# sieste/greb-climate-model

Hardware: AMD Instinct MI355X
Metric: simulated-years/sec at 96x48 grid (ensemble aggregate); diffusion HBM GB/s vs roofline (higher is better)
Workload: dtype f32; 1 GPU; 96x48 GREB ensemble, 512 members/GPU x 1 GPU, CO2 sweep 280-1120 ppm, 32 scenario years after 1 flux-correction year, dt=12h, dt_crcl=0.5h; members_per_gpu=512, arithmetic=fast, gather=none (1 GPU)

## Files before the change

greb_climate_model_amd/abi.py:

```python
from __future__ import annotations

import ctypes as C
import math

import numpy as np

NSTEP_YR = 730
NVAR_OUT = 5
F_STRICT = 1
F_MULTILAUNCH = 2
F_ROW_STRIPS = 4
F_NO_PERSISTENT = 8
F_PERSISTENT = 16
RUN_DEVICE_OUT = 1
D_REGIONS, D_ZONAL, D_ANNUAL = 1, 2, 4
D_MAX_REGIONS = 15
C_MEAN, C_SEASONS, C_TREND, C_RESPONSE = 1, 2, 4, 8
S_MEAN, S_VAR, S_RANGE, S_QUANTILES = 1, 2, 4, 8
ENS_MAX_GROUPS, ENS_MAX_PROBS, ENS_MAX_SORTED = 64, 16, 4096
L_COEF, L_RSS = 1, 2
LIN_MAX_TERMS = 64
GRAM_MAX_BLOCKS, GRAM_MAX_USED = 16, 1024
X_NAMES = ("GREB_X_NO_ICE", "GREB_X_NO_HYDRO", "GREB_X_NO_DEEP_OCEAN", "GREB_X_LW_LINEAR_VAPOR", "GREB_X_NO_CIRCULATION",
           "GREB_X_NO_VAPOR_TRANSPORT", "GREB_X_VAPOR_DIFFUSION_ONLY", "GREB_X_SST_PLUS1")
BUDGET_NAMES = ("sw", "LW_surf", "LWair_down", "LW_abs", "Q_sens", "Q_lat", "Q_lat_air", "dq_eva", "dq_rain", "dT_ocean",
                "dTo", "dTa_crcl", "dq_crcl")
NBUDGET = len(BUDGET_NAMES)
(B_SW, B_LW_SURF, B_LWAIR_DOWN, B_LW_ABS, B_Q_SENS, B_Q_LAT, B_Q_LAT_AIR, B_DQ_EVA, B_DQ_RAIN, B_DT_OCEAN, B_DTO,
 B_DTA_CRCL, B_DQ_CRCL) = range(NBUDGET)
# ... 223 lines not shown
```

greb_climate_model_amd/csrc/greb_batched.cpp:

```cpp
#include "greb_host.h"

#include <cstring>
#include <mutex>

using namespace greb;
using namespace greb::host;

#define HIP_TRY0(expr) HIP_TRY(nullptr, expr)

namespace {
int batched_common(const greb_params* p, int nx, int ny, int batch, int device) {
  if (!p || !grid_ok(nx, ny) || batch < 1) return fail(nullptr, GREB_E_INVALID, "batched: bad argument");
  return use_device("batched: ", device);
}

struct TabCache {
  struct Entry { int device; RowTables* dev; RowTables host; unsigned long long used; };
  std::mutex mu;
  std::vector<Entry> entries;
  unsigned long long clock = 0;
  static constexpr size_t kMax = 32;
} g_tab_cache;
}

// ... 87 lines not shown
  a.flux_phase = flux_phase != 0;
  a.xsw = switches ? 1u : 0u;
  if (budget) a.bsum = a.brec = budget_words;
  if (on_sets) { a.bsets = sets; a.bset_m = set_of_member; }
  if (forced || (on_sets && !flux_phase)) a.force_m = force_words;
  if (select_variant(a, variant) != hipSuccess) return fail(nullptr, GREB_E_INVALID, "step_variant: no launch carries this combination");
  return 0;
}

int greb_step_variants(unsigned* out, int capacity) {
  if (capacity < 0 || (capacity > 0 && !out)) return fail(nullptr, GREB_E_INVALID, "step_variants: bad argument");
  for (int i = 0; i < kNVariants && i < capacity; ++i) out[i] = kVariants[i];
  return kNVariants;
}

int greb_member_deal_cover(int strict, int* counts) {
  if (!counts) return fail(nullptr, GREB_E_INVALID, "member_deal_cover: bad argument");
  member_deal_cover(strict != 0, counts);
  return 0;
}

int greb_member_lds_table(int strict, int* records, int capacity) {
  if (capacity < 0 || (capacity > 0 && !records)) return fail(nullptr, GREB_E_INVALID, "member_lds_table: bad argument");
  return member_lds_table(strict != 0, records, capacity);
}

int greb_member_lds_map(int* words8) {
  if (!words8) return fail(nullptr, GREB_E_INVALID, "member_lds_map: bad argument");
  member_lds_map(words8);
  return 0;
// ... 102 lines not shown
```

greb_climate_model_amd/csrc/greb_engine.cpp:

```cpp
#include "greb_host.h"

#include <cmath>
#include <cstdio>
#include <cstring>
#include <mutex>
#include <new>

using namespace greb;
using namespace greb::host;
using StripPlan = greb_engine::StripPlan;

thread_local std::string greb::host::g_last_error;

static int nint_f(float x) { return (int)lroundf(x); }

void greb::host::compute_row_tables(const greb_params& p, float kappa, int nx, int ny, RowTables& g) {
  std::memset(&g, 0, sizeof(g));
  const float dlon = 360.f / (float)nx, dlat = 180.f / (float)ny;
  const float deg = 2.f * p.pi * 6.371e6f / 360.f;
  const float dx = dlon, dy = dlat, dyy = dy * deg;
  const float dtc = (float)p.dt_crcl;
  g.dif_ccy = kappa * dtc / (dyy * dyy);
  g.adv_ccy = dtc / dyy / 2.f;
  for (int k = 0; k < ny; ++k) {
// ... 58 lines not shown
  MemberArgs a{};
  a.nx = e->nx; a.ny = e->ny; a.np = e->np;
  a.z_topo = e->z_topo; a.glacier = e->glacier; a.sw_solar = e->sw_solar;
  a.tclim = e->tclim; a.qclim = e->qclim; a.uclim = e->uclim; a.vclim = e->vclim;
  a.mldclim = e->mldclim; a.cldclim = e->cldclim; a.swetclim = e->swetclim;
  a.toclim = e->toclim; a.z_ocean = e->z_ocean; a.wz_air = e->wz_air; a.wz_vapor = e->wz_vapor;
  a.state = e->state; a.acc = e->acc; a.corr = e->corr; a.corr_index = e->corr_index;
  a.tabs = e->tabs; a.tab_index = e->tab_index; a.phys = e->phys;
  a.nsub = nsub_of(e->p);
  a.nsub = tuning_int("GREB_DEBUG_NSUB", a.nsub);
  a.co2_flux = e->p.co2_flux;
  a.ipx = e->p.ipx; a.ipy = e->p.ipy;
  a.xsw = e->xsw_uniform ? e->xsw : 0u;
  a.xsw_m = e->xsw_uniform ? nullptr : e->xsw_dev;
  a.co2_flux_m = e->co2_flux_dev;
  a.stamps = e->stamps;
  a.dbg = tuning_int("GREB_DEBUG_PHYS", 0);
  unsigned all = GREB_X_NO_CIRCULATION;
  for (unsigned x : e->h_xsw) all &= x;
  if (all) a.nsub = 0;
  if (e->members_on_sets > 0) { a.bsets = e->bsets_dev; a.bset_m = e->bset_dev; }
  else if (e->bound[0].frec) a.bsets = e->bsets_dev;
  return a;
}

static void apply_forcing(const greb_engine* e, MemberArgs& a) {
  if (e->forced_members <= 0 && e->members_on_sets > 0) a.force_m = e->neutral_force_dev;
  if (e->forced_members <= 0) return;
  a.force_m = e->force_dev;
  a.f_space = e->f_space; a.f_season = e->f_season; a.f_solar = e->f_solar;
}
// ... 76 lines not shown
  std::lock_guard<std::mutex> lock(g_slots.mu);
  long long members = 0, taken = 0;
  SlotLedger::Entry* mine = nullptr;
  for (auto& x : g_slots.entries) {
    if (x.device != e->device) continue;
    members += x.members;
    if (x.e == e) mine = &x; else taken += x.granted;
  }
  if (!mine) return 0;
  const long long share = (long long)device_slots * mine->members / std::max<long long>(1, members);
  mine->granted = (int)std::max<long long>(0, std::min<long long>(share, device_slots - taken));
  return mine->granted;
}

static int check_circulation(greb_engine* e) {
  for (auto& kv : e->plans) {
    unsigned d[5] = {0, 0, 0, 0, 0};
    const int rc = circ_rows_status(kv.second.circ, d);
    if (rc == -1) {
      char buf[384];
      std::snprintf(buf, sizeof(buf),
                    "circulation launch given up: task %u waited more than %.1f s in sub-step %u for a neighbouring strip "
                    "(its count read %u, wanted %u) -- the launch was not resident as a whole (another process on the "
                    "device?); results are invalid, recreate the engine with GREB_F_NO_PERSISTENT",
                    d[0], kCircSpinTicks / 1e8, d[1], d[2], d[3]);
      return fail(e, GREB_E_STATE, buf);
    }
    if (rc) return fail(e, GREB_E_STATE, "circulation launch: status word unreadable");
  }
  return 0;
// ... 5 lines not shown
    static const int slots_per_cu = tuning_int("GREB_CIRC_SLOTS_PER_CU", kStepRowsSlotsPerCu);
    if (e->slots_granted < 0) e->slots_granted = ledger_grant(e, e->cus * std::min(slots_per_cu, kStepRowsSlotsPerCu));
    HIP_TRY(e, circ_rows_make_order(e->h_tabs.data(), e->h_tab_index.data(), nrun, e->ny, e->slots_granted, &p.circ));
  }
  p.form = p.circ.n == 0 ? 1 : (e->call == greb_engine::kCallAlways ? 2 : 0);
  if (p.form != 2) {
    static const int step_slots = tuning_int("GREB_STEP_SLOTS_PER_CU", kStepRowsSlotsPerCu);
    HIP_TRY(e, step_rows_make_tasks(e->h_tabs.data(), e->h_tab_index.data(), nrun, e->ny, e->cus * step_slots, &p.step_tasks,
                                    &p.n_step, p.head));
  }
  if (p.form == 0)
    for (hipEvent_t& ev : p.ev) HIP_TRY(e, hipEventCreate(&ev));
  return 0;
}

int greb::host::run_year(greb_engine* e, const MemberArgs& a, int nrun) {
  if (e->fused) {
    HIP_TRY(e, launch_member_kernel(a, nrun, e->strict, e->stream));
    return 0;
  }
  const size_t np = (size_t)e->np;
  StripPlan* plan = nullptr;
  if (e->strips && a.nsub > 0) {
    auto it = e->plans.find(nrun);
    if (it == e->plans.end()) {
      StripPlan p;
      if (int rc = make_strip_plan(e, nrun, p)) { free_plan(p); return rc; }
      it = e->plans.emplace(nrun, p).first;
    }
    plan = &it->second;
  }
  static const int steps = tuning_int("GREB_DEBUG_NSTEPS", kNT);
  bool trial = plan && plan->form == 0 && steps >= 16;
// ... 303 lines not shown
    c.p.da_ice = pick(p->da_ice, overrides[m].da_ice);
    c.p.a_no_ice = pick(p->a_no_ice, overrides[m].a_no_ice);
    c.p.a_cloud = pick(p->a_cloud, overrides[m].a_cloud);
    c.p.kappa = pick(p->kappa, overrides[m].kappa);
  }
  return create_engine("greb_engine_create", p, nx, ny, f, n_members, members.data(), device, flags, out);
}

int greb_engine_destroy(greb_engine* e) {
  if (!e) return 0;
  (void)hipSetDevice(e->device);
  void* ptrs[] = {e->z_topo, e->glacier, e->sw_solar, e->tclim, e->qclim, e->uclim, e->vclim, e->mldclim,
                  e->cldclim, e->swetclim, e->toclim, e->z_ocean, e->wz_air, e->wz_vapor, e->state, e->acc,
                  e->corr, e->corr_index, e->tab_index, e->tabs, e->phys, e->co2_dev, e->monthly_dev, e->yearly_dev,
                  e->Xa, e->Xb, e->red, e->W2, e->xsw_dev, e->co2_flux_dev, e->diag_out, e->diag_reg, e->clim_out, e->ens_out, e->lin_out, e->gram_out, e->derive_out, e->bsum, e->budget_dev,
                  e->f_space, e->f_season, e->f_solar, e->force_dev, e->bsets_dev, e->bset_dev, e->neutral_force_dev};
  for (void* q : ptrs) if (q) (void)hipFree(q);
  for (const auto& b : e->bound) if (b.frec) (void)hipFree(b.frec);
  for (size_t k = 1; k < e->bound.size(); ++k)
    for (int i = 0; i < kBoundaryFields; ++i) if (e->bound[k].own[i]) (void)hipFree(e->bound[k].dev[i]);
  for (auto& kv : e->plans) free_plan(kv.second);
  if (e->call != greb_engine::kCallNever) ledger_release(e);
  for (int i = 0; i < 2; ++i) {
    if (e->ev_done[i]) (void)hipEventDestroy(e->ev_done[i]);
    if (e->ev_free[i]) (void)hipEventDestroy(e->ev_free[i]);
  }
  if (e->copy_stream) (void)hipStreamDestroy(e->copy_stream);
  if (e->stream) (void)hipStreamDestroy(e->stream);
  delete e;
  return 0;
}
// ... 56 lines not shown
    int n = 0;
    for (const auto& b : e->bound) n += b.frec != nullptr;
    std::snprintf(buf, sizeof(buf), ", \"forcing_records\": {\"sets\": %d, \"bytes\": %zu}", n, (size_t)n * kFrBytes);
    s += buf;
  }
  {
    unsigned v;
    auto family = [&v](const MemberArgs& a) { return select_variant(a, &v) == hipSuccess ? variant_family(v) : "none"; };
    MemberArgs flux = base_args(e), scenario = base_args(e);
    flux.flux_phase = 1;
    apply_forcing(e, scenario);
    std::snprintf(buf, sizeof(buf), ", \"kernel_family\": {\"flux_correction\": \"%s\", \"scenario\": \"%s\"}", family(flux),
                  family(scenario));
    s += buf;
  }
  if (e->call != greb_engine::kCallNever) {
    std::snprintf(buf, sizeof(buf), ", \"wavefront_slots_granted\": %d, \"circulation\": [", e->slots_granted);
    s += buf;
    bool first = true;
    for (const auto& kv : e->plans) {
      const StripPlan& p = kv.second;
      std::snprintf(buf, sizeof(buf), "%s{\"members_run\": %d, \"tasks_of_one_launch_per_call\": %d, \"form\": \"%s\", \"trial_ms_per_3_steps\": [%.4f, %.4f]}",
                    first ? "" : ", ", kv.first, p.circ.n,
                    p.circ.n == 0 ? "one launch per sub-step (slots)" : (p.form == 2 ? "one launch per call" : (p.form == 1 ? "one launch per sub-step" : "undecided")),
                    p.ms_substep, p.ms_call);
      s += buf;
      first = false;
    }
    s += "]";
  }
// ... 18 lines not shown
}

int greb_engine_set_corrections(greb_engine* e, int member, const float* corr, const float* state5) {
  if (!e || member < -1 || member >= e->nm) return fail(e, GREB_E_INVALID, "set_corrections: bad argument");
  HIP_TRY(e, hipSetDevice(e->device));
  const size_t n = (size_t)3 * kNT * e->np, s5 = (size_t)5 * e->np;
  const int m0 = member < 0 ? 0 : member, m1 = member < 0 ? e->nm : member + 1;
  for (int m = m0; m < m1; ++m) {
    const size_t ci = e->shared_corr ? 0 : (size_t)m;
    if (corr && (ci == (size_t)m || m == m0)) HIP_TRY(e, hipMemcpy(e->corr + ci * n, corr, n * sizeof(float), hipMemcpyHostToDevice));
    if (state5) HIP_TRY(e, hipMemcpy(e->state + (size_t)m * s5, state5, s5 * sizeof(float), hipMemcpyHostToDevice));
  }
  return 0;
}

int greb_engine_set_state(greb_engine* e, int member, const float* state5) {
  if (!state5) return fail(e, GREB_E_INVALID, "set_state: bad argument");
  return greb_engine_set_corrections(e, member, nullptr, state5);
}

}
```

greb_climate_model_amd/csrc/greb_host.h:

```cpp
#pragma once
#include "../../include/greb_engine.h"

#include <hip/hip_runtime.h>

#include <functional>
#include <map>
#include <string>
#include <vector>

#include "greb_kernels.h"

struct greb_engine {
  greb_params p{};
  int nx = 0, ny = 0, np = 0, nm = 0, device = 0;
  bool strict = false;
  unsigned xsw = 0;
  std::vector<unsigned> h_xsw;
  bool xsw_uniform = true;
  unsigned* xsw_dev = nullptr;
  float* co2_flux_dev = nullptr;
  int n_phys_sets = 1;
  bool shared_corr = true;
  bool fused = true;
  float *Xa = nullptr, *Xb = nullptr, *red = nullptr, *W2 = nullptr;
// ... 47 lines not shown
  int cus = 0;
  int slots_granted = -1;
  struct StripPlan {
    greb::RowsTask* step_tasks = nullptr;
    int n_step = 0;
    greb::RowsTask head[greb::kStepHeadTasks] = {};
    greb::CircOrder circ;
    int form = 0;
    float ms_substep = 0.f, ms_call = 0.f;
    hipEvent_t ev[3] = {nullptr, nullptr, nullptr};
  };
  std::map<int, StripPlan> plans;
  std::vector<greb::Phys> h_phys;
  long long it_flux = 0;
  long long it_scnr = 0;
  unsigned long long* stamps = nullptr;
  std::string last_error;
};

namespace greb {
namespace host {

extern thread_local std::string g_last_error;
int fail(greb_engine* e, int code, const std::string& msg);

#define HIP_STEP(e, who, what, expr)                                                          \
  do {                                                                                        \
    hipError_t _err = (expr);                                                                 \
    if (_err != hipSuccess)                                                                   \
      return fail((e), (int)_err, std::string(who) + (what) + ": " + hipGetErrorString(_err)); \
// ... 86 lines not shown
```

greb_climate_model_amd/csrc/greb_kernels.h:

```cpp
#pragma once
#include <hip/hip_runtime.h>

#include <cstdlib>
#include <utility>
#include <vector>

#include "greb_device.h"

namespace greb {

constexpr int kNT = 730;

#ifdef GREB_TUNING
inline int tuning_int(const char* name, int dflt) {
  const char* e = getenv(name);
  return e ? atoi(e) : dflt;
}
#else
constexpr int tuning_int(const char*, int dflt) { return dflt; }
#endif

constexpr int kMaxDynamicLds = 160 * 1024;

struct MemberForcing {
// ... 13 lines not shown
constexpr int kMaxBoundarySets = 16;

constexpr int kFrNx = 96, kFrNy = 48;
enum { kFrZtopo, kFrGlacier, kFrZocean, kFrWzAir, kFrStaticFields,
       kFrTclim = kFrStaticFields, kFrCld, kFrMld, kFrMldPrev, kFrSwet, kFrWind, kFrFields };
constexpr int kFrStepFields = kFrFields - kFrStaticFields;
constexpr unsigned forcing_record_offset(int row, int field, int lon) {
  return field < kFrStaticFields ? ((unsigned)row * kFrStaticFields + (unsigned)field) * kFrNx + (unsigned)lon
                                 : ((unsigned)row * kFrStepFields + (unsigned)(field - kFrStaticFields)) * kFrNx + (unsigned)lon;
}
constexpr unsigned kFrStaticFloats = forcing_record_offset(kFrNy, 0, 0), kFrStepFloats = forcing_record_offset(kFrNy, kFrStaticFields, 0);
constexpr size_t kFrBytes = ((size_t)kFrStaticFloats + (size_t)kNT * kFrStepFloats) * sizeof(float);
static_assert(forcing_record_offset(0, kFrFields - 1, 0) * sizeof(float) <= 4095 && forcing_record_offset(0, kFrStaticFields - 1, 0) * sizeof(float) <= 4095,
              "a field's offset must fit the immediate of a global load");
static_assert(kFrBytes < (1ull << 31), "offsets into a record are 32-bit");

struct MemberArgs {
  int nx, ny, np;
  const float *z_topo, *glacier, *sw_solar;
  const float *tclim, *qclim, *uclim, *vclim, *mldclim, *cldclim, *swetclim;
  const float *toclim, *z_ocean, *wz_air, *wz_vapor;
  float* state;
  float* acc;
  float* corr;
  const int* corr_index;
  const RowTables* tabs;
  const int* tab_index;
  const Phys* phys;
  int flux_phase;
  long long it0;
// ... 12 lines not shown
  unsigned xsw;
  unsigned long long* stamps;
  int dbg;
  const unsigned* xsw_m;
  const float* co2_flux_m;
  float* bsum;
  float* brec;
  int brec_years;
  int brec_year0;
  const MemberForcing* force_m;
  const float* f_space;
  const float* f_season;
  const float* f_solar;
  const BoundarySet* bsets;
  const int* bset_m;
};

constexpr int kSetTableEntries = kMaxBoundarySets + 1;
constexpr size_t kSetTableBytes = kSetTableEntries * (sizeof(BoundarySet) + sizeof(const float*));
inline const float** set_table_records(BoundarySet* table) { return (const float**)(table + kSetTableEntries); }

enum { kBsw, kBLWsurf, kBLWdown, kBLWabs, kBQsens, kBQlat, kBQlatAir, kBdqEva, kBdqRain, kBdTocean, kBdTo, kBdTaCrcl, kBdqCrcl, kNBudget };

enum : unsigned { kVFlux = 1, kVExp = 2, kVBudget = 4, kVForce = 8, kVBound = 16 };
constexpr bool variant_valid(unsigned v) {
  const bool flux = v & kVFlux, exp = v & kVExp, budget = v & kVBudget, force = v & kVForce, bound = v & kVBound;
  return v < 32u && !(budget && flux) && (!force || (exp && !flux)) && (!bound || (exp && (flux || force)));
}
constexpr unsigned kVariants[] = {0u, kVFlux, kVExp, kVFlux | kVExp, kVBudget, kVExp | kVBudget, kVExp | kVForce,
                                  kVExp | kVBudget | kVForce, kVFlux | kVExp | kVBound, kVExp | kVForce | kVBound,
// ... 18 lines not shown
  return (v & kVBound) ? "boundary" : (v & kVForce) ? "forcing" : (v & kVExp) ? "switches" : "default";
}
template <template <bool, unsigned> class Family, size_t... I>
auto pick_variant(bool strict, unsigned v, std::index_sequence<I...>) {
  decltype(Family<false, 0u>::kernel()) k = nullptr;
  ((kVariants[I] == v ? (void)(k = strict ? Family<true, kVariants[I]>::kernel() : Family<false, kVariants[I]>::kernel()) : (void)0), ...);
  return k;
}
template <template <bool, unsigned> class Family>
auto pick_variant(bool strict, unsigned v) { return pick_variant<Family>(strict, v, std::make_index_sequence<kNVariants>{}); }

bool member_layout_supported(const RowTables& tab, int nx, int ny);
void member_deal_cover(bool strict, int* counts);
int member_lds_table(bool strict, int* out, int capacity);
void member_lds_map(int* words8);
hipError_t launch_member_kernel(const MemberArgs& a, int n_members, bool strict, hipStream_t s);
hipError_t launch_pack_forcing(const BoundarySet& b, float* rec, hipStream_t s);
hipError_t launch_circulation_g96(const float* X, const float* wz, const float* u, const float* v, float* dX,
                                  const RowTables* tab_dev, int batch, int nsub, bool strict, hipStream_t s);

hipError_t launch_diffusion(const float* T1, const float* wz, float* dX, const RowTables* tab_dev,
                            const RowTables& tab_host, int nx, int ny, int batch, bool strict, hipStream_t s);
bool rows_supported(const RowTables& t, int nx, int ny);
struct RowsTask { int field, rows; };
constexpr int kRowsUp = 1 << 20;
struct RowsTuning {
  int chain_target;
  int chain_span;
  int parts[4];
  int level_tasks[4];
};
// ... 72 lines not shown
```

greb_climate_model_amd/csrc/greb_member.hip:

```cpp
#include <cstdlib>

#include "greb_kernels.h"
#include "greb_pair.h"
#include "greb_physics_step.h"
#include "greb_stencil.h"

namespace greb {

constexpr int NX = 96, NY = 48, NQ = 24, NP = 4608;
constexpr int kThreads = 512;
constexpr int RS = 2 * NX + 16;
constexpr int XB = (NY + 2) * RS;
constexpr int kOffX = RS;
constexpr int kOffW = 2 * XB + RS;
constexpr int kOffWX = 3 * XB;
constexpr int kOffWY = kOffWX + NP;
constexpr int kOffRowK = kOffWY + NP;
constexpr int kRowKCsDif = 7;
constexpr int kLdsFloats = kOffRowK + NY * kRowKWords;
constexpr size_t kLdsBytes = (size_t)kLdsFloats * sizeof(float);

bool member_layout_supported(const RowTables& t, int nx, int ny) {
  if (nx != NX || ny != NY) return false;
  for (int k = 0; k < NY; ++k) {
// ... 612 lines not shown
            const float y = vq[j].v[e];
            vq[j].v[e] = (k == 1 ? y > 0.f : y < 0.f) ? 3.f * y : y;
          }
        }
      }
      st4(lds + kOffWX + 4 * i, uq[j]); st4(lds + kOffWY + 4 * i, vq[j]);
    }
  }
  (void)tab;
}

template <bool STRICT>
struct Circ {
  __device__ __forceinline__ void init(lfloat* lds, const float* wz_air, const float* wz_vapor,
                                       const RowTables* __restrict__ tab) {
    for (int i = threadIdx.x; i < 6 * RS; i += kThreads) {
      const int g = i / RS, o = i % RS;
      lds[(g >> 1) * XB + (g & 1) * (NY + 1) * RS + o] = 0.f;
    }
    stage_row_consts(lds + kOffRowK, *tab, 0, NY);
    if (!STRICT)
      for (int k = threadIdx.x; k < NY; k += blockDim.x)
        lds[kOffRowK + k * kRowKWords + kRowKCsDif] = lds[kOffRowK + k * kRowKWords] * 0.05f;
    for (int i = threadIdx.x; i < NP / 4; i += kThreads)
      st8(lds + kOffW + (i / NQ) * RS, i % NQ, zip(ld4(wz_air + 4 * i), ld4(wz_vapor + 4 * i)));
  }

  template <int WAVE, bool NOT_CALM>
  __device__ __forceinline__ void role_loop(lfloat* lds, int cur, int nsub, int lane, int dbg, bool calm_runtime
#ifdef GREB_TUNING
                                            , bool stamp, unsigned long long& busy
#endif
  ) {
    const bool calm_q = NOT_CALM ? false : calm_runtime;
    constexpr bool kPolar = is_polar_wave<STRICT>(WAVE);
    BulkTasks tasks;
    BulkSigns signs;
    QuadChain quad;
    if constexpr (!kPolar) tasks = make_tasks<STRICT, WAVE>(lane);
// ... 68 lines not shown
    st4(dX + fo + 4 * i, f4{{a.v[0] - b.v[0], a.v[1] - b.v[1], a.v[2] - b.v[2], a.v[3] - b.v[3]}});
  }
}

hipError_t launch_circulation_g96(const float* X, const float* wz, const float* u, const float* v, float* dX,
                                  const RowTables* tab_dev, int batch, int nsub, bool strict, hipStream_t s) {
  auto kern = strict ? circulation_g96_kernel<true> : circulation_g96_kernel<false>;
  hipError_t e = hipFuncSetAttribute(reinterpret_cast<const void*>(kern),
                                     hipFuncAttributeMaxDynamicSharedMemorySize, (int)kLdsBytes);
  if (e != hipSuccess) return e;
  hipLaunchKernelGGL(kern, dim3(batch), dim3(kThreads), kLdsBytes, s, X, wz, u, v, dX, tab_dev, nsub,
                     tuning_int("GREB_DEBUG_SKIP", 0));
  return hipGetLastError();
}

template <bool STRICT, unsigned V>
__global__ __launch_bounds__(kThreads) void member_kernel(MemberArgs a) {
  constexpr bool FLUX = V & kVFlux, EXP = V & kVExp, BUDGET = V & kVBudget, FORCE = V & kVForce, BOUND = V & kVBound;
  extern __shared__ __align__(16) float lds_raw[];
  lfloat* lds = (lfloat*)lds_raw;
  const int m = blockIdx.x, tid = threadIdx.x;
  float* state = a.state + (size_t)m * 5 * NP;
  float* acc = a.acc + (size_t)m * 6 * NP;
  float* corr = a.corr + (size_t)a.corr_index[m] * 3 * kNT * NP;
  const RowTables* tab = a.tabs + a.tab_index[m];

#ifdef GREB_TUNING
  for (int i = 0; i < (a.dbg >> 8) * (m & 7); ++i) __builtin_amdgcn_s_sleep(16);
#endif
  Circ<STRICT> circ;
  const int bset = member_bset<BOUND>(a, m);
  {
    const BoundPtr B = member_boundary<BOUND>(a, bset);
    circ.init(lds, BOUND ? (const float*)B->wz_air : a.wz_air, BOUND ? (const float*)B->wz_vapor : a.wz_vapor, tab);
  }
  for (int i = tid; i < NP / 4; i += kThreads)
    st8(lds + kOffX + (i / NQ) * RS, i % NQ, zip(ld4(state + NP + 4 * i), ld4(state + 3 * NP + 4 * i)));
  int cur = 0;
  const unsigned xsw = EXP ? member_switches(a, m) : 0u;
  const int nsub = (EXP && (xsw & kXNoCirc)) ? 0 : a.nsub;
  const bool q_dif_only = EXP && (xsw & kXQDiffOnly) && !(xsw & kXNoQTransport);
  const float co2_flux = FLUX ? (a.co2_flux_m ? a.co2_flux_m[m] : a.co2_flux) : 0.f;
  __syncthreads();
#ifdef GREB_TUNING
  const bool stamp = a.stamps != nullptr;
  unsigned long long st_wind = 0, st_circ = 0, st_busy = 0, st_phys = 0;
  const unsigned long long st_c0 = stamp ? __builtin_amdgcn_s_memtime() : 0, st_r0 = stamp ? __builtin_amdgcn_s_memrealtime() : 0;
#define GREB_STAMP(var) const unsigned long long var = stamp ? __builtin_amdgcn_s_memtime() : 0
#else
#define GREB_STAMP(var)
#endif

#pragma unroll 1
  for (int s = 0; s < a.nsteps; ++s) {
    const long long it = a.it0 + s;
    const StepClock ck = step_clock<FLUX>(a, it, NP);
    const int ityr = ck.ityr, yr_rel = ck.yr_rel;
    const size_t off = ck.off;

    GREB_STAMP(t_a);
    {
      const BoundPtr B = member_boundary<BOUND>(a, bset);
      stage_winds<STRICT, EXP && !STRICT>(lds, (BOUND ? (const float*)B->uclim : a.uclim) + off,
                                          (BOUND ? (const float*)B->vclim : a.vclim) + off, tab);
    }
    __syncthreads();
    GREB_STAMP(t_b);

#ifdef GREB_TUNING
// ... 63 lines not shown
        }
      }
    }
    __syncthreads();
#ifdef GREB_TUNING
    if (stamp) {
      const unsigned long long t_d = __builtin_amdgcn_s_memtime();
      st_wind += t_b - t_a; st_circ += t_c - t_b; st_phys += t_d - t_c;
    }
#endif
  }
#ifdef GREB_TUNING
  if (stamp && (tid & 63) == 0) {
    unsigned long long* o = a.stamps + ((size_t)m * (kThreads / 64) + (tid >> 6)) * 8;
    o[0] = __builtin_amdgcn_s_memtime() - st_c0; o[1] = __builtin_amdgcn_s_memrealtime() - st_r0;
    o[2] = st_wind; o[3] = st_circ; o[4] = st_busy; o[5] = st_phys; o[6] = (unsigned long long)a.nsteps; o[7] = (unsigned long long)nsub;
  }
#endif
}

static_assert(kFrNx == NX && kFrNy == NY, "the forcing record is the fused kernel's grid");
__global__ __launch_bounds__(256) void pack_forcing_kernel(BoundarySet b, float* __restrict__ rec) {
  const unsigned i = blockIdx.x * 256u + threadIdx.x;
  if (i >= (unsigned)kNT * NP) return;
  const unsigned step = i / NP, p = i - step * NP, row = p / NX, lon = p - row * NX;
  const unsigned prev = step > 0 ? step - 1 : kNT - 1;
  const float zt = b.z_topo[p];
  if (step == 0) {
    float* o = rec + forcing_record_offset((int)row, 0, (int)lon);
    o[forcing_record_offset(0, kFrZtopo, 0)] = zt;
    o[forcing_record_offset(0, kFrGlacier, 0)] = b.glacier[p];
    o[forcing_record_offset(0, kFrZocean, 0)] = b.z_ocean[p];
    o[forcing_record_offset(0, kFrWzAir, 0)] = b.wz_air[p];
// ... 3 lines not shown
  o[forcing_record_offset(0, kFrCld, 0)] = b.cldclim[i];
  o[forcing_record_offset(0, kFrMld, 0)] = b.mldclim[i];
  o[forcing_record_offset(0, kFrMldPrev, 0)] = b.mldclim[(size_t)prev * NP + p];
  o[forcing_record_offset(0, kFrSwet, 0)] = b.swetclim[i];
  o[forcing_record_offset(0, kFrWind, 0)] = wind_speed<false>(b.uclim[i], b.vclim[i], zt);
}

hipError_t launch_pack_forcing(const BoundarySet& b, float* rec, hipStream_t s) {
  hipLaunchKernelGGL(pack_forcing_kernel, dim3((kNT * NP + 255) / 256), dim3(256), 0, s, b, rec);
  return hipGetLastError();
}

template <bool STRICT, unsigned V>
struct MemberFamily { static auto kernel() { return &member_kernel<STRICT, V>; } };

hipError_t launch_member_kernel(const MemberArgs& a, int n_members, bool strict, hipStream_t s) {
  if (a.nx != NX || a.ny != NY) return hipErrorInvalidValue;
  if (!strict && !a.bsets) return hipErrorInvalidValue;
  unsigned v;
  if (hipError_t e = select_variant(a, &v); e != hipSuccess) return e;
  const auto kern = pick_variant<MemberFamily>(strict, v);
  if (!kern) return hipErrorInvalidValue;
  hipError_t e = hipFuncSetAttribute(reinterpret_cast<const void*>(kern),
                                     hipFuncAttributeMaxDynamicSharedMemorySize, (int)kLdsBytes);
  if (e != hipSuccess) return e;
  hipLaunchKernelGGL(kern, dim3(n_members), dim3(kThreads), kLdsBytes, s, a);
  return hipGetLastError();
}

}
```

greb_climate_model_amd/csrc/greb_stencil.h:

```cpp
#pragma once
#include "greb_chain6.h"
#include "greb_device.h"

namespace greb {

__device__ __forceinline__ void wave_lds_sync() {
  asm volatile("s_waitcnt lgkmcnt(0)" ::: "memory");
  __builtin_amdgcn_wave_barrier();
}

struct Rows {
  const lfloat* base;
  int r0, nx;
  __device__ __forceinline__ const lfloat* row(int k) const { return base + (k - r0) * nx; }
};

struct QuadIn {
  float T[12], w[12];
  f4 T0, w0, Tm2, Tm1, Tp1, Tp2, wm2, wm1, wp1, wp2;
};


struct RowK {
  float dif_cc;
  float adv_cc;
  float dif_ccy, adv_ccy;
  int sub;
  int dif_time2, adv_time2;
};
constexpr int kRowKWords = 8;
__device__ __forceinline__ void stage_row_consts(lfloat* dst, const RowTables& tab, int k_begin, int k_end) {
  for (int k = k_begin + threadIdx.x; k < k_end; k += blockDim.x) {
    const int sub = tab.subcycled[k];
    lfloat* d = dst + (k - k_begin) * kRowKWords;
    d[0] = sub ? tab.dif_ccx2[k] : tab.dif_ccx[k];
    d[1] = sub ? tab.adv_ccx2[k] : tab.adv_ccx[k];
    d[2] = tab.dif_ccy; d[3] = tab.adv_ccy;
    d[4] = __int_as_float(sub); d[5] = __int_as_float(tab.dif_time2[k]); d[6] = __int_as_float(tab.adv_time2[k]);
    d[7] = 0.f;
  }
}
__device__ __forceinline__ RowK row_consts(const lfloat* src, int k) {
  const f4 a = ld4(src + k * kRowKWords), b = ld4(src + k * kRowKWords + 4);
  RowK r;
  r.dif_cc = a.v[0]; r.adv_cc = a.v[1]; r.dif_ccy = a.v[2]; r.adv_ccy = a.v[3];
  r.sub = __float_as_int(b.v[0]); r.dif_time2 = __float_as_int(b.v[1]); r.adv_time2 = __float_as_int(b.v[2]);
  return r;
// ... 325 lines not shown
```

greb_climate_model_amd/engine.py:

```python
from __future__ import annotations

import ctypes as C
import json
import os

import numpy as np

from . import abi, build, workload

_lib = None


class GrebError(RuntimeError):
    def __init__(self, code: int, msg: str):
        super().__init__(f"greb engine error {code}: {msg}")
        self.code = code


_lib_path = build.LIB


def use_tuning_build() -> None:
    global _lib_path
    if _lib is not None:
# ... 36 lines not shown
           "greb_clim_create", "greb_clim_destroy", "greb_clim_add_year_dev", "greb_clim_finish_dev", "greb_engine_run_clim",
           "greb_ens_create", "greb_ens_destroy", "greb_ens_reduce_dev", "greb_engine_run_ens",
           "greb_lin_create", "greb_lin_destroy", "greb_lin_reduce_dev", "greb_engine_run_lin",
           "greb_forcing_record_offset", "greb_forcing_record_field_bytes", "greb_forcing_record_step_floats",
           "greb_forcing_record_bytes", "greb_forcing_record_field_name", "greb_engine_get_forcing_record",
           "greb_forcing_record_field_static", "greb_forcing_record_static_floats",
           "greb_diag_create_vars", "greb_clim_create_vars", "greb_budget_combine_dev", "greb_engine_run_budget_diag",
           "greb_engine_run_budget_clim", "greb_engine_run_budget_ens", "greb_engine_run_budget_lin",
           "greb_gram_create", "greb_gram_destroy", "greb_gram_reduce_dev", "greb_engine_run_gram", "greb_engine_run_budget_gram",
           "greb_cross_create", "greb_cross_destroy", "greb_cross_add_year_dev", "greb_cross_finish_dev", "greb_engine_run_cross",
           "greb_engine_run_budget_cross",
           "greb_reg_create", "greb_reg_destroy", "greb_reg_add_year_dev", "greb_reg_finish_dev", "greb_engine_run_reg",
           "greb_engine_run_budget_reg",
           "greb_derive_create", "greb_derive_destroy", "greb_derive_uses_budget", "greb_derive_apply_dev",
           "greb_engine_run_derived_diag", "greb_engine_run_derived_clim", "greb_engine_run_derived_ens", "greb_engine_run_derived_lin",
           "greb_engine_run_derived_gram", "greb_engine_run_derived_cross", "greb_engine_run_derived_reg"]


def _check(rc: int, h=None):
    if rc != 0:
        msg = lib().greb_engine_last_error(h)
        raise GrebError(rc, msg.decode() if msg else "")


def device_info(device: int = 0) -> dict:
    return json.loads(lib().greb_device_info(device).decode())


def budget_name(i: int) -> str | None:
    f = lib().greb_budget_name
    f.restype = C.c_char_p
# ... 85 lines not shown
                 (abi.F_ROW_STRIPS if row_strips else 0) |
                 (0 if persistent is None else (abi.F_PERSISTENT if persistent else abi.F_NO_PERSISTENT)))
        if members is not None:
            rc = L.greb_engine_create_members(C.byref(self.params), inp.nx, inp.ny, C.byref(fields), n_members,
                                              member_configs(self.params, members), device, flags, C.byref(self.h))
        else:
            rc = L.greb_engine_create(C.byref(self.params), inp.nx, inp.ny, C.byref(fields), n_members, ov, device, flags,
                                      C.byref(self.h))
        if rc != 0:
            msg = L.greb_engine_last_error(self.h).decode()
            if self.h:
                L.greb_engine_destroy(self.h)
                self.h = None
            raise GrebError(rc, msg)

    def describe(self) -> dict:
        f = lib().greb_engine_describe
        f.restype = C.c_char_p
        return json.loads(f(self.h).decode())

    def close(self):
        if getattr(self, "h", None):
            lib().greb_engine_destroy(self.h)
            self.h = None

    def __del__(self):
        try:
            self.close()
        except Exception:
            pass
# ... 262 lines not shown
def substep_launch_order(params, nx, ny, n_members, kappa=None):
    params = params if params is not None else params_default()
    kap = None if kappa is None else np.ascontiguousarray(kappa, np.float32)
    kp = None if kap is None else kap.ctypes.data_as(C.POINTER(C.c_float))
    f = lib().greb_substep_launch_order
    n = f(C.byref(params), nx, ny, n_members, kp, None, None, None, 0)
    if n < 0:
        _check(n)
    out = [np.zeros(n, np.int32) for _ in range(3)]
    if n:
        ptr = [a.ctypes.data_as(C.POINTER(C.c_int)) for a in out]
        assert f(C.byref(params), nx, ny, n_members, kp, *ptr, n) == n
    return out


def member_deal_cover(strict=False):
    out = np.zeros((48, 24), np.int32)
    _check(lib().greb_member_deal_cover(int(bool(strict)), out.ctypes.data_as(C.POINTER(C.c_int))))
    return out


LDS_KINDS = ("column", "side", "wind", "store", "const")


def member_lds_map():
    w = (C.c_int * 8)()
    _check(lib().greb_member_lds_map(w))
    return dict(zip(("RS", "X0", "X1", "W", "WX", "WY", "ROWK", "END"), (int(x) for x in w)))


# ... 67 lines not shown
```

include/greb_engine.h:

```cpp
#ifndef GREB_ENGINE_H
#define GREB_ENGINE_H

#include <stddef.h>
#include <stdint.h>

#ifdef __cplusplus
extern "C" {
#endif

#define GREB_NSTEP_YR 730
#define GREB_NVAR_OUT 5

#define GREB_E_INVALID   (-1)
#define GREB_E_NOGPU     (-2)
#define GREB_E_STATE     (-3)
#define GREB_E_UNSUPPORTED (-4)

typedef struct greb_params {
  float pi, sig, rho_ocean, rho_land, rho_air, cp_ocean, cp_land, cp_air, eps;
  float d_ocean, d_land, d_air, ct_sens, da_ice, a_no_ice, a_cloud;
  float Tl_ice1, Tl_ice2, To_ice1, To_ice2;
  float co_turb, kappa, ce, cq_latent, cq_rain, z_air, z_vapor, r_qviwv;
  float p_emi[10];
  float co2_flux;
// ... 309 lines not shown
                               void* stream);
int greb_release_caches(void);
int greb_diffusion_launch_order(const greb_params* p, int nx, int ny, int batch, int* field, int* k0, int* k1, int* up,
                                int capacity);
int greb_substep_launch_order(const greb_params* p, int nx, int ny, int n_members, const float* kappa, int* field, int* k0,
                              int* k1, int capacity);

int greb_circulation_launch_plan(const greb_params* p, int nx, int ny, int n_members, const float* kappa, int slots,
                                 int* field, int* k0, int* k1, int* chain, int* dep4, int capacity);

int greb_member_deal_cover(int strict, int* counts);

int greb_member_lds_table(int strict, int* records, int capacity);
int greb_member_lds_map(int* words8);

#define GREB_FORCING_RECORD_FIELDS 10
int greb_forcing_record_field_static(int field);
long long greb_forcing_record_offset(int row, int field, int lon);
long long greb_forcing_record_field_bytes(int field);
long long greb_forcing_record_static_floats(void);
long long greb_forcing_record_step_floats(void);
long long greb_forcing_record_bytes(void);
const char* greb_forcing_record_field_name(int field);
int greb_engine_get_forcing_record(greb_engine* e, int set, int step, float* out);

#define GREB_V_FLUX 1u
#define GREB_V_SWITCHES 2u
#define GREB_V_BUDGET 4u
#define GREB_V_FORCING 8u
#define GREB_V_BOUNDARY 16u
// ... 15 lines not shown
```

Measured before the change: 5886 simulated-years/s.

## Deal member-year chunks to persistent workgroups through a device work queue

When there are more members than compute units, the fused member kernel now launches one workgroup per CU instead of one per member. Each workgroup pops (member, chunk) items from a global atomic queue, runs that slice of the year's steps, then pushes the member's next chunk. Chunks follow a halving schedule so the work left at the end of a launch comes in small pieces, meant to even out the tail where some CUs sit idle. In exchange, every chunk reloads the member's state and LDS constants, adds atomics, spin-waits and a per-launch queue reset copy, and a host status check reports a workgroup that waits too long.

```diff
diff --git a/greb_climate_model_amd/abi.py b/greb_climate_model_amd/abi.py
--- a/greb_climate_model_amd/abi.py
+++ b/greb_climate_model_amd/abi.py
@@ -13,6 +13,7 @@
 F_NO_PERSISTENT = 8
 F_PERSISTENT = 16
 RUN_DEVICE_OUT = 1
+MAX_CHUNKS, CHUNKS_HALVING, CHUNKS_EQUAL, CHUNKS_QUARTERS = 10, 0, 1, 2
 D_REGIONS, D_ZONAL, D_ANNUAL = 1, 2, 4
 D_MAX_REGIONS = 15
 C_MEAN, C_SEASONS, C_TREND, C_RESPONSE = 1, 2, 4, 8
diff --git a/greb_climate_model_amd/csrc/greb_batched.cpp b/greb_climate_model_amd/csrc/greb_batched.cpp
--- a/greb_climate_model_amd/csrc/greb_batched.cpp
+++ b/greb_climate_model_amd/csrc/greb_batched.cpp
@@ -125,6 +125,20 @@
   return kNVariants;
 }
 
+int greb_member_chunk_table(int schedule, int nsteps, int* end, int capacity) {
+  if (schedule < 0 || schedule >= kNChunkSchedules || nsteps < 1 || capacity < 0 || (capacity > 0 && !end))
+    return fail(nullptr, GREB_E_INVALID, "member_chunk_table: bad argument");
+  const ChunkTable t = chunk_table(schedule, nsteps);
+  for (int c = 0; c < t.n && c < capacity; ++c) end[c] = t.end[c];
+  return t.n;
+}
+
+long long greb_member_queue_capacity(int members, int schedule, int nsteps) {
+  if (schedule < 0 || schedule >= kNChunkSchedules || nsteps < 1 || members < 1 || members > kMaxDealtMembers)
+    return fail(nullptr, GREB_E_INVALID, "member_queue_capacity: bad argument");
+  return (long long)members * chunk_table(schedule, nsteps).n;
+}
+
 int greb_member_deal_cover(int strict, int* counts) {
   if (!counts) return fail(nullptr, GREB_E_INVALID, "member_deal_cover: bad argument");
   member_deal_cover(strict != 0, counts);
diff --git a/greb_climate_model_amd/csrc/greb_engine.cpp b/greb_climate_model_amd/csrc/greb_engine.cpp
--- a/greb_climate_model_amd/csrc/greb_engine.cpp
+++ b/greb_climate_model_amd/csrc/greb_engine.cpp
@@ -96,7 +96,7 @@
   a.xsw = e->xsw_uniform ? e->xsw : 0u;
   a.xsw_m = e->xsw_uniform ? nullptr : e->xsw_dev;
   a.co2_flux_m = e->co2_flux_dev;
-  a.stamps = e->stamps;
+  a.stamps = e->stamps; a.stamp_members = e->nm;
   a.dbg = tuning_int("GREB_DEBUG_PHYS", 0);
   unsigned all = GREB_X_NO_CIRCULATION;
   for (unsigned x : e->h_xsw) all &= x;
@@ -203,6 +203,19 @@
 }
 
 static int check_circulation(greb_engine* e) {
+  if (e->deal_status) {
+    unsigned d[4] = {0, 0, 0, 0};
+    if (hipMemcpy(d, e->deal_status, sizeof(d), hipMemcpyDeviceToHost) != hipSuccess)
+      return fail(e, GREB_E_STATE, "dealt member launch: status word unreadable");
+    if (d[0]) {
+      char buf[256];
+      std::snprintf(buf, sizeof(buf),
+                    "dealt member launch given up: a workgroup waited more than %.1f s for item %u of its queue; results are "
+                    "invalid, recreate the engine (greb_engine_set_dealing(e, -1, 0, 0) runs it without the queue)",
+                    kCircSpinTicks / 1e8, d[1]);
+      return fail(e, GREB_E_STATE, buf);
+    }
+  }
   for (auto& kv : e->plans) {
     unsigned d[5] = {0, 0, 0, 0, 0};
     const int rc = circ_rows_status(kv.second.circ, d);
@@ -238,9 +251,44 @@
   return 0;
 }
 
+static int deal_prepare(greb_engine* e, MemberArgs& a, int nrun, int* workgroups) {
+  if (e->deal_workgroups < 0 || a.nsteps < 1 || nrun > kMaxDealtMembers) return 0;
+  if (e->cus <= 0) HIP_TRY(e, hipDeviceGetAttribute(&e->cus, hipDeviceAttributeMultiprocessorCount, e->device));
+  const int w = e->deal_workgroups > 0 ? e->deal_workgroups : e->cus;
+  if (w < 1 || (nrun <= w && !e->deal_force)) return 0;
+  const ChunkTable t = chunk_table(e->deal_schedule, a.nsteps);
+  const size_t capacity = (size_t)nrun * (size_t)t.n, words = kQItems + capacity;
+  if (!e->deal_status) {
+    DevBuf<unsigned> st;
+    HIP_TRY(e, st.alloc(4));
+    HIP_TRY(e, hipMemset(st.get(), 0, 4 * sizeof(unsigned)));
+    e->deal_status = st.release();
+  }
+  if (e->deal_members != nrun || e->deal_chunks != t.n) {
+    HIP_TRY(e, hipStreamSynchronize(e->stream));
+    std::vector<unsigned> image(words, 0u);
+    image[kQTail] = (unsigned)nrun;
+    for (int m = 0; m < nrun; ++m) image[kQItems + (size_t)m] = ((unsigned)m << 4) + 1u;
+    DevBuf<unsigned> q, img;
+    HIP_TRY(e, q.alloc(words));
+    HIP_TRY(e, img.upload(image.data(), words));
+    adopt(e->deal_queue, q);
+    adopt(e->deal_image, img);
+    e->deal_members = nrun; e->deal_chunks = t.n;
+  }
+  HIP_TRY(e, hipMemcpyAsync(e->deal_queue, e->deal_image, words * sizeof(unsigned), hipMemcpyDeviceToDevice, e->stream));
+  a.queue = e->deal_queue; a.q_status = e->deal_status; a.q_capacity = (unsigned)capacity; a.chunks = t;
+  *workgroups = w;
+  ++e->deal_launches;
+  return 0;
+}
+
 int greb::host::run_year(greb_engine* e, const MemberArgs& a, int nrun) {
   if (e->fused) {
-    HIP_TRY(e, launch_member_kernel(a, nrun, e->strict, e->stream));
+    MemberArgs b = a;
+    int workgroups = 0;
+    if (int rc = deal_prepare(e, b, nrun, &workgroups)) return rc;
+    HIP_TRY(e, launch_member_kernel(b, nrun, e->strict, e->stream, workgroups));
     return 0;
   }
   const size_t np = (size_t)e->np;
@@ -574,7 +622,8 @@
                   e->cldclim, e->swetclim, e->toclim, e->z_ocean, e->wz_air, e->wz_vapor, e->state, e->acc,
                   e->corr, e->corr_index, e->tab_index, e->tabs, e->phys, e->co2_dev, e->monthly_dev, e->yearly_dev,
                   e->Xa, e->Xb, e->red, e->W2, e->xsw_dev, e->co2_flux_dev, e->diag_out, e->diag_reg, e->clim_out, e->ens_out, e->lin_out, e->gram_out, e->derive_out, e->bsum, e->budget_dev,
-                  e->f_space, e->f_season, e->f_solar, e->force_dev, e->bsets_dev, e->bset_dev, e->neutral_force_dev};
+                  e->f_space, e->f_season, e->f_solar, e->force_dev, e->bsets_dev, e->bset_dev, e->neutral_force_dev,
+                  e->deal_queue, e->deal_image, e->deal_status};
   for (void* q : ptrs) if (q) (void)hipFree(q);
   for (const auto& b : e->bound) if (b.frec) (void)hipFree(b.frec);
   for (size_t k = 1; k < e->bound.size(); ++k)
@@ -661,6 +710,11 @@
                   family(scenario));
     s += buf;
   }
+  if (e->fused) {
+    std::snprintf(buf, sizeof(buf), ", \"dealing\": {\"workgroups\": %d, \"schedule\": %d, \"forced\": %s, \"dealt_launches\": %lld}",
+                  e->deal_workgroups, e->deal_schedule, e->deal_force ? "true" : "false", e->deal_launches);
+    s += buf;
+  }
   if (e->call != greb_engine::kCallNever) {
     std::snprintf(buf, sizeof(buf), ", \"wavefront_slots_granted\": %d, \"circulation\": [", e->slots_granted);
     s += buf;
@@ -709,6 +763,12 @@
   return 0;
 }
 
+int greb_engine_set_dealing(greb_engine* e, int workgroups, int schedule, int force) {
+  if (!e || schedule < 0 || schedule >= kNChunkSchedules) return fail(e, GREB_E_INVALID, "set_dealing: bad argument");
+  e->deal_workgroups = workgroups; e->deal_schedule = schedule; e->deal_force = force != 0;
+  return 0;
+}
+
 int greb_engine_set_state(greb_engine* e, int member, const float* state5) {
   if (!state5) return fail(e, GREB_E_INVALID, "set_state: bad argument");
   return greb_engine_set_corrections(e, member, nullptr, state5);
diff --git a/greb_climate_model_amd/csrc/greb_host.h b/greb_climate_model_amd/csrc/greb_host.h
--- a/greb_climate_model_amd/csrc/greb_host.h
+++ b/greb_climate_model_amd/csrc/greb_host.h
@@ -85,6 +85,14 @@
   std::vector<greb::Phys> h_phys;
   long long it_flux = 0;
   long long it_scnr = 0;
+  int deal_workgroups = 0;
+  int deal_schedule = greb::kChunksHalving;
+  bool deal_force = false;
+  unsigned* deal_queue = nullptr;
+  unsigned* deal_image = nullptr;
+  unsigned* deal_status = nullptr;
+  int deal_members = 0, deal_chunks = 0;
+  long long deal_launches = 0;
   unsigned long long* stamps = nullptr;
   std::string last_error;
 };
diff --git a/greb_climate_model_amd/csrc/greb_kernels.h b/greb_climate_model_amd/csrc/greb_kernels.h
--- a/greb_climate_model_amd/csrc/greb_kernels.h
+++ b/greb_climate_model_amd/csrc/greb_kernels.h
@@ -51,6 +51,24 @@
 static_assert(forcing_record_offset(0, kFrFields - 1, 0) * sizeof(float) <= 4095 && forcing_record_offset(0, kFrStaticFields - 1, 0) * sizeof(float) <= 4095,
               "a field's offset must fit the immediate of a global load");
 static_assert(kFrBytes < (1ull << 31), "offsets into a record are 32-bit");
+
+constexpr int kMaxChunks = 10;
+struct ChunkTable { int n; int end[kMaxChunks]; };
+enum { kChunksHalving = 0, kChunksEqual = 1, kChunksQuarters = 2, kNChunkSchedules };
+inline ChunkTable chunk_table(int schedule, int nsteps) {
+  constexpr int kHalving[7] = {365, 548, 639, 685, 708, 720, 730};
+  constexpr int kQuarters[8] = {183, 365, 548, 639, 685, 708, 720, 730};
+  ChunkTable t{};
+  const int n = schedule == kChunksEqual ? kMaxChunks : (schedule == kChunksQuarters ? 8 : 7);
+  for (int c = 0; c < n; ++c) {
+    const long long e = schedule == kChunksEqual ? (long long)nsteps * (c + 1) / n
+                                                 : (long long)nsteps * (schedule == kChunksQuarters ? kQuarters[c] : kHalving[c]) / 730;
+    if (e > (t.n ? t.end[t.n - 1] : 0)) t.end[t.n++] = (int)e;
+  }
+  return t;
+}
+enum { kQHead = 0, kQTail = 1, kQItems = 4 };
+constexpr int kMaxDealtMembers = 1 << 27;
 
 struct MemberArgs {
   int nx, ny, np;
@@ -93,6 +111,11 @@
   const float* f_solar;
   const BoundarySet* bsets;
   const int* bset_m;
+  unsigned* queue;
+  unsigned* q_status;
+  unsigned q_capacity;
+  ChunkTable chunks;
+  int stamp_members;
 };
 
 constexpr int kSetTableEntries = kMaxBoundarySets + 1;
@@ -141,7 +164,7 @@
 void member_deal_cover(bool strict, int* counts);
 int member_lds_table(bool strict, int* out, int capacity);
 void member_lds_map(int* words8);
-hipError_t launch_member_kernel(const MemberArgs& a, int n_members, bool strict, hipStream_t s);
+hipError_t launch_member_kernel(const MemberArgs& a, int n_members, bool strict, hipStream_t s, int workgroups = 0);
 hipError_t launch_pack_forcing(const BoundarySet& b, float* rec, hipStream_t s);
 hipError_t launch_circulation_g96(const float* X, const float* wz, const float* u, const float* v, float* dX,
                                   const RowTables* tab_dev, int batch, int nsub, bool strict, hipStream_t s);
diff --git a/greb_climate_model_amd/csrc/greb_member.hip b/greb_climate_model_amd/csrc/greb_member.hip
--- a/greb_climate_model_amd/csrc/greb_member.hip
+++ b/greb_climate_model_amd/csrc/greb_member.hip
@@ -650,15 +650,17 @@
 struct Circ {
   __device__ __forceinline__ void init(lfloat* lds, const float* wz_air, const float* wz_vapor,
                                        const RowTables* __restrict__ tab) {
-    for (int i = threadIdx.x; i < 6 * RS; i += kThreads) {
+    int tid = threadIdx.x;
+    asm volatile("" : "+v"(tid));
+    for (int i = tid; i < 6 * RS; i += kThreads) {
       const int g = i / RS, o = i % RS;
       lds[(g >> 1) * XB + (g & 1) * (NY + 1) * RS + o] = 0.f;
     }
-    stage_row_consts(lds + kOffRowK, *tab, 0, NY);
+    stage_row_consts(lds + kOffRowK, *tab, 0, NY, tid);
     if (!STRICT)
-      for (int k = threadIdx.x; k < NY; k += blockDim.x)
+      for (int k = tid; k < NY; k += blockDim.x)
         lds[kOffRowK + k * kRowKWords + kRowKCsDif] = lds[kOffRowK + k * kRowKWords] * 0.05f;
-    for (int i = threadIdx.x; i < NP / 4; i += kThreads)
+    for (int i = tid; i < NP / 4; i += kThreads)
       st8(lds + kOffW + (i / NQ) * RS, i % NQ, zip(ld4(wz_air + 4 * i), ld4(wz_vapor + 4 * i)));
   }
 
@@ -757,12 +759,88 @@
   return hipGetLastError();
 }
 
+constexpr int kLdsItemWord = kLdsFloats;
+constexpr size_t kLdsBytesLaunch = kLdsBytes + 16;
+static_assert(kLdsBytesLaunch <= 160 * 1024, "the item word must fit the CU's LDS beside the member");
+
+__device__ __forceinline__ int item_member(unsigned item) { return (int)((item - 1u) >> 4); }
+__device__ __forceinline__ int item_chunk(unsigned item) { return (int)((item - 1u) & 15u); }
+__device__ __forceinline__ __attribute__((address_space(3))) unsigned* item_words(lfloat* lds) {
+  return (__attribute__((address_space(3))) unsigned*)(lds + kLdsItemWord);
+}
+__device__ __forceinline__ unsigned item_word(lfloat* lds, int i) {
+  return (unsigned)__builtin_amdgcn_readfirstlane((int)*(volatile __attribute__((address_space(3))) unsigned*)(item_words(lds) + i));
+}
+__device__ __forceinline__ unsigned pop_item(const MemberArgs& a, lfloat* lds) {
+  __attribute__((address_space(3))) unsigned* word = item_words(lds) + 2;
+  if (threadIdx.x == 0) {
+    unsigned item = 0u;
+    const unsigned idx = __hip_atomic_fetch_add(a.queue + kQHead, 1u, __ATOMIC_RELAXED, __HIP_MEMORY_SCOPE_AGENT);
+    if (idx < a.q_capacity) {
+      const unsigned long long t0 = __builtin_amdgcn_s_memrealtime();
+      for (;;) {
+        item = __hip_atomic_load(a.queue + kQItems + idx, __ATOMIC_RELAXED, __HIP_MEMORY_SCOPE_AGENT);
+        if (item != 0u) break;
+        if (__hip_atomic_load(a.q_status, __ATOMIC_RELAXED, __HIP_MEMORY_SCOPE_AGENT) != 0u) break;
+        if (__builtin_amdgcn_s_memrealtime() - t0 > kCircSpinTicks) {
+          __hip_atomic_store(a.q_status + 1, idx, __ATOMIC_RELAXED, __HIP_MEMORY_SCOPE_AGENT);
+          __hip_atomic_store(a.q_status, 1u, __ATOMIC_RELAXED, __HIP_MEMORY_SCOPE_AGENT);
+          break;
+        }
+        __builtin_amdgcn_s_sleep(64);
+      }
+    }
+    *word = item;
+  }
+  __syncthreads();
+  const unsigned item = (unsigned)__builtin_amdgcn_readfirstlane((int)*word);
+  __builtin_amdgcn_fence(__ATOMIC_ACQUIRE, "agent");
+  return item;
+}
+
+__device__ __forceinline__ void push_next(const MemberArgs& a, unsigned item) {
+  __builtin_amdgcn_fence(__ATOMIC_RELEASE, "agent");
+  __syncthreads();
+  if (threadIdx.x == 0 && item_chunk(item) + 1 < a.chunks.n) {
+    __builtin_amdgcn_fence(__ATOMIC_RELEASE, "agent");
+    const unsigned slot = __hip_atomic_fetch_add(a.queue + kQTail, 1u, __ATOMIC_RELAXED, __HIP_MEMORY_SCOPE_AGENT);
+    if (slot < a.q_capacity)
+      __hip_atomic_store(a.queue + kQItems + slot, item + 1u, __ATOMIC_RELEASE, __HIP_MEMORY_SCOPE_AGENT);
+  }
+}
+
 template <bool STRICT, unsigned V>
-__global__ __launch_bounds__(kThreads) void member_kernel(MemberArgs a) {
+__global__ __launch_bounds__(kThreads) void member_kernel(MemberArgs a_launch) {
   constexpr bool FLUX = V & kVFlux, EXP = V & kVExp, BUDGET = V & kVBudget, FORCE = V & kVForce, BOUND = V & kVBound;
   extern __shared__ __align__(16) float lds_raw[];
   lfloat* lds = (lfloat*)lds_raw;
-  const int m = blockIdx.x, tid = threadIdx.x;
+  const int tid = threadIdx.x;
+  const bool dealt = a_launch.queue != nullptr;
+#pragma unroll 1
+  for (;;) {
+  const __attribute__((address_space(4))) MemberArgs* a_trip =
+      (const __attribute__((address_space(4))) MemberArgs*)__builtin_amdgcn_kernarg_segment_ptr();
+  asm volatile("" : "+s"(a_trip));
+  const MemberArgs& a = *(const MemberArgs*)a_trip;
+  int m = blockIdx.x, s0 = 0;
+  {
+    int s1 = a.nsteps;
+    unsigned item = ((unsigned)m << 4) + 1u;
+    if (dealt) {
+      item = pop_item(a, lds);
+      if (item == 0u) break;
+      m = item_member(item);
+#pragma unroll
+      for (int c = 0; c < kMaxChunks; ++c) {
+        if (c + 1 == item_chunk(item)) s0 = a.chunks.end[c];
+        if (c == item_chunk(item)) s1 = a.chunks.end[c];
+      }
+    }
+    if (tid == 0) { item_words(lds)[0] = item; item_words(lds)[1] = (unsigned)s1; }
+  }
+#ifdef GREB_TUNING
+  const unsigned long long tl_r0 = a.stamps ? __builtin_amdgcn_s_memrealtime() : 0, tl_c0 = a.stamps ? __builtin_amdgcn_s_memtime() : 0;
+#endif
   float* state = a.state + (size_t)m * 5 * NP;
   float* acc = a.acc + (size_t)m * 6 * NP;
   float* corr = a.corr + (size_t)a.corr_index[m] * 3 * kNT * NP;
@@ -777,8 +855,12 @@
     const BoundPtr B = member_boundary<BOUND>(a, bset);
     circ.init(lds, BOUND ? (const float*)B->wz_air : a.wz_air, BOUND ? (const float*)B->wz_vapor : a.wz_vapor, tab);
   }
-  for (int i = tid; i < NP / 4; i += kThreads)
-    st8(lds + kOffX + (i / NQ) * RS, i % NQ, zip(ld4(state + NP + 4 * i), ld4(state + 3 * NP + 4 * i)));
+  {
+    int t = tid;
+    asm volatile("" : "+v"(t));
+    for (int i = t; i < NP / 4; i += kThreads)
+      st8(lds + kOffX + (i / NQ) * RS, i % NQ, zip(ld4(state + NP + 4 * i), ld4(state + 3 * NP + 4 * i)));
+  }
   int cur = 0;
   const unsigned xsw = EXP ? member_switches(a, m) : 0u;
   const int nsub = (EXP && (xsw & kXNoCirc)) ? 0 : a.nsub;
@@ -795,7 +877,7 @@
 #endif
 
 #pragma unroll 1
-  for (int s = 0; s < a.nsteps; ++s) {
+  for (int s = s0; s < (int)item_word(lds, 1); ++s) {
     const long long it = a.it0 + s;
     const StepClock ck = step_clock<FLUX>(a, it, NP);
     const int ityr = ck.ityr, yr_rel = ck.yr_rel;
@@ -889,9 +971,22 @@
   if (stamp && (tid & 63) == 0) {
     unsigned long long* o = a.stamps + ((size_t)m * (kThreads / 64) + (tid >> 6)) * 8;
     o[0] = __builtin_amdgcn_s_memtime() - st_c0; o[1] = __builtin_amdgcn_s_memrealtime() - st_r0;
-    o[2] = st_wind; o[3] = st_circ; o[4] = st_busy; o[5] = st_phys; o[6] = (unsigned long long)a.nsteps; o[7] = (unsigned long long)nsub;
-  }
-#endif
+    o[2] = st_wind; o[3] = st_circ; o[4] = st_busy; o[5] = st_phys; o[6] = (unsigned long long)((int)item_word(lds, 1) - s0); o[7] = (unsigned long long)nsub;
+  }
+  if (stamp && tid == 0) {
+    unsigned hw, xcc;
+    asm volatile("s_getreg_b32 %0, hwreg(HW_REG_HW_ID)" : "=s"(hw));
+    asm volatile("s_getreg_b32 %0, hwreg(HW_REG_XCC_ID)" : "=s"(xcc));
+    const int chunk = item_chunk(item_word(lds, 0));
+    unsigned long long* o = a.stamps + (size_t)a.stamp_members * (kThreads / 64) * 8 + ((size_t)m * kMaxChunks + chunk) * 8;
+    o[0] = tl_r0; o[1] = __builtin_amdgcn_s_memrealtime(); o[2] = ((unsigned long long)xcc << 32) | hw;
+    o[3] = __builtin_amdgcn_s_memtime() - tl_c0; o[4] = st_c0 - tl_c0; o[5] = (unsigned long long)s0; o[6] = (unsigned long long)item_word(lds, 1);
+    o[7] = (unsigned long long)blockIdx.x;
+  }
+#endif
+  if (!dealt) break;
+  push_next(a, item_word(lds, 0));
+  }
 }
 
 static_assert(kFrNx == NX && kFrNy == NY, "the forcing record is the fused kernel's grid");
@@ -925,17 +1020,20 @@
 template <bool STRICT, unsigned V>
 struct MemberFamily { static auto kernel() { return &member_kernel<STRICT, V>; } };
 
-hipError_t launch_member_kernel(const MemberArgs& a, int n_members, bool strict, hipStream_t s) {
+hipError_t launch_member_kernel(const MemberArgs& a, int n_members, bool strict, hipStream_t s, int workgroups) {
   if (a.nx != NX || a.ny != NY) return hipErrorInvalidValue;
+  if (a.queue && (workgroups < 1 || !a.q_status || a.chunks.n < 1 || a.chunks.n > kMaxChunks || n_members > kMaxDealtMembers ||
+                  a.q_capacity != (unsigned)n_members * (unsigned)a.chunks.n || a.chunks.end[a.chunks.n - 1] != a.nsteps))
+    return hipErrorInvalidValue;
   if (!strict && !a.bsets) return hipErrorInvalidValue;
   unsigned v;
   if (hipError_t e = select_variant(a, &v); e != hipSuccess) return e;
   const auto kern = pick_variant<MemberFamily>(strict, v);
   if (!kern) return hipErrorInvalidValue;
   hipError_t e = hipFuncSetAttribute(reinterpret_cast<const void*>(kern),
-                                     hipFuncAttributeMaxDynamicSharedMemorySize, (int)kLdsBytes);
+                                     hipFuncAttributeMaxDynamicSharedMemorySize, (int)kLdsBytesLaunch);
   if (e != hipSuccess) return e;
-  hipLaunchKernelGGL(kern, dim3(n_members), dim3(kThreads), kLdsBytes, s, a);
+  hipLaunchKernelGGL(kern, dim3(a.queue ? workgroups : n_members), dim3(kThreads), kLdsBytesLaunch, s, a);
   return hipGetLastError();
 }
 
diff --git a/greb_climate_model_amd/csrc/greb_stencil.h b/greb_climate_model_amd/csrc/greb_stencil.h
--- a/greb_climate_model_amd/csrc/greb_stencil.h
+++ b/greb_climate_model_amd/csrc/greb_stencil.h
@@ -29,8 +29,8 @@
   int dif_time2, adv_time2;
 };
 constexpr int kRowKWords = 8;
-__device__ __forceinline__ void stage_row_consts(lfloat* dst, const RowTables& tab, int k_begin, int k_end) {
-  for (int k = k_begin + threadIdx.x; k < k_end; k += blockDim.x) {
+__device__ __forceinline__ void stage_row_consts(lfloat* dst, const RowTables& tab, int k_begin, int k_end, int tid = threadIdx.x) {
+  for (int k = k_begin + tid; k < k_end; k += blockDim.x) {
     const int sub = tab.subcycled[k];
     lfloat* d = dst + (k - k_begin) * kRowKWords;
     d[0] = sub ? tab.dif_ccx2[k] : tab.dif_ccx[k];
diff --git a/greb_climate_model_amd/engine.py b/greb_climate_model_amd/engine.py
--- a/greb_climate_model_amd/engine.py
+++ b/greb_climate_model_amd/engine.py
@@ -74,7 +74,8 @@
            "greb_engine_run_budget_reg",
            "greb_derive_create", "greb_derive_destroy", "greb_derive_uses_budget", "greb_derive_apply_dev",
            "greb_engine_run_derived_diag", "greb_engine_run_derived_clim", "greb_engine_run_derived_ens", "greb_engine_run_derived_lin",
-           "greb_engine_run_derived_gram", "greb_engine_run_derived_cross", "greb_engine_run_derived_reg"]
+           "greb_engine_run_derived_gram", "greb_engine_run_derived_cross", "greb_engine_run_derived_reg",
+           "greb_engine_set_dealing", "greb_member_chunk_table", "greb_member_queue_capacity"]
 
 
 def _check(rc: int, h=None):
@@ -190,6 +191,9 @@
                 self.h = None
             raise GrebError(rc, msg)
 
+    def set_dealing(self, workgroups: int = 0, schedule: int = abi.CHUNKS_HALVING, force: bool = False) -> None:
+        _check(lib().greb_engine_set_dealing(self.h, int(workgroups), int(schedule), int(bool(force))), self.h)
+
     def describe(self) -> dict:
         f = lib().greb_engine_describe
         f.restype = C.c_char_p
@@ -482,6 +486,23 @@
     return out
 
 
+def member_chunk_table(schedule: int = abi.CHUNKS_HALVING, nsteps: int = abi.NSTEP_YR) -> list[int]:
+    end = (C.c_int * abi.MAX_CHUNKS)()
+    n = lib().greb_member_chunk_table(int(schedule), int(nsteps), end, abi.MAX_CHUNKS)
+    if n < 0:
+        _check(n)
+    return [int(end[i]) for i in range(n)]
+
+
+def member_queue_capacity(members: int, schedule: int = abi.CHUNKS_HALVING, nsteps: int = abi.NSTEP_YR) -> int:
+    f = lib().greb_member_queue_capacity
+    f.restype = C.c_longlong
+    n = int(f(int(members), int(schedule), int(nsteps)))
+    if n < 0:
+        _check(n)
+    return n
+
+
 def member_deal_cover(strict=False):
     out = np.zeros((48, 24), np.int32)
     _check(lib().greb_member_deal_cover(int(bool(strict)), out.ctypes.data_as(C.POINTER(C.c_int))))
diff --git a/include/greb_engine.h b/include/greb_engine.h
--- a/include/greb_engine.h
+++ b/include/greb_engine.h
@@ -347,6 +347,14 @@
 int greb_member_lds_table(int strict, int* records, int capacity);
 int greb_member_lds_map(int* words8);
 
+#define GREB_MAX_CHUNKS 10
+#define GREB_CHUNKS_HALVING 0
+#define GREB_CHUNKS_EQUAL   1
+#define GREB_CHUNKS_QUARTERS 2
+int greb_engine_set_dealing(greb_engine* e, int workgroups, int schedule, int force);
+int greb_member_chunk_table(int schedule, int nsteps, int* end, int capacity);
+long long greb_member_queue_capacity(int members, int schedule, int nsteps);
+
 #define GREB_FORCING_RECORD_FIELDS 10
 int greb_forcing_record_field_static(int field);
 long long greb_forcing_record_offset(int row, int field, int lon);
```

New measurement: 6000 simulated-years/s, median of 6. 1.02x the previous value.
